# soulslicer/probabilistic-depth

Hardware: AMD Instinct MI355X
Metric: depth-volumes/sec (D=64, 256x512) (higher is better)
Workload: dtype f32 (fp16-pair products on MFMA, fp32 accumulate)

## Files before the change

probabilistic-depth_amd/csrc/sweep_dist.hip:

```cpp
#include <hip/hip_runtime.h>

#include <atomic>
#include <climits>
#include <cstdlib>

#include "dist_layout.hpp"
#include "epipolar_probe.hpp"
#include "geometry.hpp"
#include "kernels.hpp"
#include "sweep_workspace.hpp"
#include "wave_util.hpp"

#include "sweep_dist_knobs.hpp"

namespace pdepth {

namespace {

using namespace wv;
typedef _Float16 h8 __attribute__((ext_vector_type(8)));
typedef _Float16 h2 __attribute__((ext_vector_type(2)));
typedef int v2i __attribute__((ext_vector_type(2)));

constexpr int DIST_MAXV = 8;

struct DistArgs {
    SweepArgs a;
    const char* packed;
    const float* stats;
    int* queue;
    int* qcnt;
    int qstride;
    int tiles_x, ntile;
    int one_each;
    int nblk;
    int nonce;
};
#define KARG(type, field) kernarg_at<type>(offsetof(DistArgs, field))


__device__ __forceinline__ float dist_exp(float x) {
    return __builtin_amdgcn_exp2f((x < -1000.0f ? -1000.0f : x) * 1.44269502162933349609375f);
}

template <int MAXB, int NAC>
struct __attribute__((aligned(16))) DistLds {
    static constexpr int XSTRIDE = MAXB * 16 + 4;
    float Ys[16 * XSTRIDE];
    float Qs[(MAXB + 3) / 4 * 256 + 8];
    _Float16 Bs[NAC * 4 * 16 * 8];
    float rp[4 * 16 * 2];
    float mus[dist::MAX_C + 8];
    float xf[DIST_MAXV * 12];
    float cst[8];
    float red[4 * 16 * 4];
    float dcl[128];
    int ctab[2][64 * 2];
    int ired[2][2];
    int brow[MAXB + 2];
    v4i rec[2];
    int iflag;
    unsigned char wide[64];
};

template <int NCHK, int NH>
__global__ __launch_bounds__(256, NH == 1 ? DIST_OCC1 : DIST_OCC2) void sweep_dist_kernel(DistArgs da) {
    constexpr int NAC = 2 * NCHK + 1;
    constexpr int MP = NCHK + 1;
    constexpr int MAXB = NH == 1 ? DIST_MAXB1 : DIST_MAXB2;
    constexpr int NC = 4 * NH;
    constexpr int QPL = 8 * NCHK + 3;
    constexpr int NS = NH == 1 ? DIST_SETS1 : DIST_SETS2;
    typedef DistLds<MAXB, NAC> Lds;
    constexpr int XSTRIDE = Lds::XSTRIDE;
    __shared__ Lds L;
#ifdef DIST_STAMPS
    unsigned long long stamp_acc[12] = {0, 0, 0, 0, 0, 0, 0, 0, 0, 0, 0, 0};
    unsigned long long stamp_t = __builtin_amdgcn_s_memtime();
#endif
    if (poison_on_foreign_layout(da.a, da.queue, LAYOUT_DIST16)) return;
    const int tid = threadIdx.x;
    constexpr int QT = 64 * DIST_QUEUE_WAVE;
    static_assert(DIST_QUEUE_WAVE >= 0 && DIST_QUEUE_WAVE < 4, "a workgroup has four waves");

    {
        const float* dc = KARG(const float*, a.d_candi);
        const int D = KARG(int, a.D);
        for (int k = tid; k < 64 * NH; k += 256) L.dcl[k] = dc[min(k, D - 1)];
    }
    if (tid < 128) { L.ctab[0][tid] = (tid & 1) ? INT_MIN : INT_MAX; L.ctab[1][tid] = (tid & 1) ? INT_MIN : INT_MAX; }
    if (tid < 64) L.wide[tid] = 1;
    if (tid < 2) { L.ired[tid][0] = INT_MAX; L.ired[tid][1] = INT_MIN; }
    __syncthreads();
    if ((int)(tid >> 2) < min(KARG(int, a.B), 64) && epipolar_probe_is_steep(da.a, tid >> 2, tid & 3)) L.wide[tid >> 2] = 0;

    const int xcd = blockIdx.x & 7;
    if (blockIdx.x == 0 && tid == 0) KARG(int*, queue)[DIST_NONCE_SLOT] = KARG(int, nonce);
    auto band_tiles_of = [&](int q) { const int nt = KARG(int, ntile); return (nt >> 3) + (q < (nt & 7) ? 1 : 0); };
    auto band_first_of = [&](int q) {
        const int nt = KARG(int, ntile), qq = nt >> 3, rr8 = nt & 7;
        return q < rr8 ? q * (qq + 1) : rr8 * (qq + 1) + (q - rr8) * qq;
    };
    auto items_of = [&](int q) { return 4 * band_tiles_of(q) * KARG(int, a.B); };
    int own_done = 0;
    auto steal = [&]() -> int {
        int* qcnt = KARG(int*, qcnt);
        const int qs = KARG(int, qstride);
#pragma unroll 1
        for (int j = 1; j < 8; ++j) {
            const int q = (opaque_s(xcd) + j) & 7, nq = items_of(q);
            if (__hip_atomic_load(&qcnt[q * qs], __ATOMIC_RELAXED, __HIP_MEMORY_SCOPE_AGENT) >= nq) continue;
            const int got = atomicAdd(&qcnt[q * qs], 1);
            if (got < nq) return (q << 28) | got;
        }
        return -1;
    };
    auto resolve = [&](int got) -> int {
        const int n_own = items_of(xcd);
        if (!own_done && got < n_own) return (opaque_s(xcd) << 28) | got;
        own_done = 1;
        return steal();
    };
    auto fdiv = [](int nn, int dd) { return (int)(((float)nn + 0.5f) * __builtin_amdgcn_rcpf((float)dd)); };
    auto decode = [&](int item, int& b_, int& tx_, int& ty_, int& sub_) {
        const int ntile = KARG(int, ntile), tiles_x = KARG(int, tiles_x), H = KARG(int, a.H);
        const int qq = ntile >> 3, rr8 = ntile & 7;
        const bool small_idx = (long long)ntile * 4 * KARG(int, a.B) < (1ll << 22);
        const int tiles_y_ = (H + 3) / 4;
        const int q_ = item >> 28, iq = item & 0x0fffffff, band_tiles = band_tiles_of(q_);
        const int tidx = iq >> 2;
        sub_ = iq & 3;
        b_ = small_idx ? fdiv(tidx, band_tiles) : tidx / band_tiles;
        const int ti = tidx - b_ * band_tiles;
        int tile = band_first_of(q_) + ti;
        if (rr8 == 0 && tiles_y_ % 16 == 0 && tiles_y_ * tiles_x == ntile) {
            const int hb_rows = tiles_y_ / 16, half_tiles = hb_rows * tiles_x;
            const int second = ti >= half_tiles ? 1 : 0, tih = ti - second * half_tiles;
            const int hbi = (q_ < 4) == (second == 0) ? q_ : 8 + q_;
            const int cc = small_idx ? fdiv(tih, hb_rows) : tih / hb_rows, r_ = tih - cc * hb_rows;
            tile = (hbi * hb_rows + r_) * tiles_x + cc;
        } else if (rr8 == 0 && qq % tiles_x == 0) {
            const int band_rows = qq / tiles_x, tc = small_idx ? fdiv(ti, band_rows) : ti / band_rows;
            tile = (q_ * band_rows + (ti - tc * band_rows)) * tiles_x + tc;
        }
        ty_ = small_idx ? fdiv(tile, tiles_x) : tile / tiles_x;
        tx_ = tile - ty_ * tiles_x;
        if (DIST_REV_BATCH && KARG(const float*, a.src) != nullptr) b_ = KARG(int, a.B) - 1 - b_;
    };
#define ONE_EACH (KARG(int, one_each) != 0)
    __syncthreads();

    int state = 0;
    int n_direct = 0;
    int got_own = (tid == QT && !ONE_EACH) ? atomicAdd(&KARG(int*, qcnt)[xcd * KARG(int, qstride)], 1) : (int)(blockIdx.x >> 3);
    int next_item = -1;
    auto resolve_next = [&]() { if (opaque_v((int)threadIdx.x) == QT) next_item = ONE_EACH ? -1 : resolve(got_own); };
    constexpr int REC_WIDE = 1, REC_BELOW = 2, REC_FIRST = 4;
    auto publish = [&](int slot, int item) {
        v4i r = v4i{item, 0, 0, 0};
        if (item >= 0) {
            int b, tx, ty, sub;
            decode(item, b, tx, ty, sub);
            const bool wide = b < 64 ? L.wide[b] != 0 : false;
            const int x0 = wide ? tx * 16 : tx * 16 + 8 * (sub & 1), y0 = wide ? ty * 4 + sub : ty * 4 + 2 * (sub >> 1);
            r.y = b;
            r.z = (y0 << 16) | x0;
            r.w = (wide ? REC_WIDE : 0) | (y0 >= KARG(int, a.H) ? REC_BELOW : 0) | ((tx | ty | sub) == 0 ? REC_FIRST : 0);
        }
        L.rec[slot] = r;
    };
    constexpr bool EARLY = DIST_DECODE_EARLY != 0;
    constexpr bool POP_EARLY = EARLY && DIST_PREFETCH == 0;
    auto record_next = [&](bool decode = true, bool pop = true) {
        if (opaque_v((int)threadIdx.x) == QT) {
            if (decode) publish(state & 1, next_item);
            if (pop && POP_EARLY && !ONE_EACH && !own_done) got_own = atomicAdd(&KARG(int*, qcnt)[xcd * KARG(int, qstride)], 1);
        }
    };
    auto publish_next = [&]() {
        if (opaque_v((int)threadIdx.x) == QT) {
            if (!EARLY) publish(state & 1, next_item);
            if (!POP_EARLY && !ONE_EACH && !own_done) got_own = atomicAdd(&KARG(int*, qcnt)[xcd * KARG(int, qstride)], 1);
        }
    };
    constexpr bool PF = DIST_PREFETCH != 0;
    constexpr int ZW = 64 + 128 * NCHK;
    static_assert(4 * ZW + 128 <= (int)(sizeof(Lds::Qs) / sizeof(float)), "the prefetch zone does not fit L.Qs");
    auto dma_pixels = [&](int wave, int b, int p4) {
        const int H = KARG(int, a.H), W = KARG(int, a.W), C = KARG(int, a.C), HW = H * W;
        const int kq = (opaque_v((int)threadIdx.x) & 63) >> 4;
        const __amdgpu_buffer_rsrc_t rray =
            __builtin_amdgcn_make_buffer_rsrc((void*)(KARG(const float*, a.rays) + (size_t)b * 3 * HW), 0, 3 * HW * 4, 0x00020000);
        const __amdgpu_buffer_rsrc_t rref = __builtin_amdgcn_make_buffer_rsrc(
            (void*)(KARG(const float*, a.ref) + (size_t)b * KARG(long long, a.ref_bstride)), 0, C * HW * 4, 0x00020000);
        dma_b32(rray, lds_addr_of(&L.Qs[wave * ZW]), kq < 3 ? kq * HW * 4 + p4 : OOB, 0);
#pragma unroll
        for (int mm = 0; mm < NCHK; ++mm)
#pragma unroll
            for (int j = 0; j < 2; ++j) {
                const int cr = 8 * wave + 4 * j + kq;
                dma_b32(rref, lds_addr_of(&L.Qs[wave * ZW + 64 + 128 * mm + 64 * j]), cr < C - 32 * mm ? cr * HW * 4 + p4 : OOB, 32 * mm * HW * 4);
            }
        if (wave == 0) {
#pragma unroll
            for (int j = 0; j < 2; ++j) {
                const int cr = 4 * j + kq;
                dma_b32(rref, lds_addr_of(&L.Qs[4 * ZW + 64 * j]), cr < C - 32 * NCHK ? cr * HW * 4 + p4 : OOB, 32 * NCHK * HW * 4);
            }
        }
    };
    auto prefetch_next = [&](int wave) {
        const v4i nrec = L.rec[state & 1];
        if (__builtin_amdgcn_readfirstlane(nrec.x) < 0) return;
        const int fl = __builtin_amdgcn_readfirstlane(nrec.w);
        if (fl & REC_BELOW) return;
        const int b = __builtin_amdgcn_readfirstlane(nrec.y), xy = __builtin_amdgcn_readfirstlane(nrec.z);
        const int H = KARG(int, a.H), W = KARG(int, a.W);
        const int n = opaque_v((int)threadIdx.x) & 15;
        const int x = (xy & 0xffff) + ((fl & REC_WIDE) ? n : (n & 7));
        const int y = (xy >> 16) + ((fl & REC_WIDE) ? 0 : (n >> 3));
        dma_pixels(wave, b, (min(y, H - 1) * W + min(x, W - 1)) * 4);
        state |= 4;
    };
    if (tid == QT) {
        publish(0, ONE_EACH ? (got_own < items_of(xcd) ? (xcd << 28) | got_own : -1) : resolve(got_own));
        if (!ONE_EACH && !own_done) got_own = atomicAdd(&KARG(int*, qcnt)[xcd * KARG(int, qstride)], 1);
    }
    PDEPTH_LDS_BARRIER();
#define PDEPTH_POP_WAIT(n) __builtin_amdgcn_s_waitcnt(0x0f70 | (n))
    PDEPTH_POP_WAIT(0);

    for (;;) {
        const v4i rec = L.rec[state & 1];
        state ^= 1;
        const int pf = state & 4;
        state ^= pf;
        if (__builtin_amdgcn_readfirstlane(rec.x) < 0) break;
        DSTAMP(0)
        const int wave = opaque_s(__builtin_amdgcn_readfirstlane((int)threadIdx.x >> 6));
        const int b = __builtin_amdgcn_readfirstlane(rec.y), xy0 = __builtin_amdgcn_readfirstlane(rec.z), recfl = __builtin_amdgcn_readfirstlane(rec.w);
        const int H = KARG(int, a.H), W = KARG(int, a.W), V = KARG(int, a.V), C = KARG(int, a.C), D = KARG(int, a.D);
        const bool wide = (recfl & REC_WIDE) != 0;

        {
            if (recfl & REC_BELOW) {
                resolve_next();
                if (EARLY) record_next();
                publish_next();
                PDEPTH_LDS_BARRIER();
                PDEPTH_POP_WAIT(0);
                continue;
            }
            const int tid = opaque_v((int)threadIdx.x), lane = tid & 63;
            const int n = lane & 15, kq = lane >> 4, tq = wave * 4 + kq;
            const int a32 = (lane ^ 32) << 2;
            const int HW = H * W;
            int p;
            bool xlive;
            float ray[3], rv[MP][2];
            {
                const __amdgpu_buffer_rsrc_t rray =
                    __builtin_amdgcn_make_buffer_rsrc((void*)(KARG(const float*, a.rays) + (size_t)b * 3 * HW), 0, 3 * HW * 4, 0x00020000);
                const __amdgpu_buffer_rsrc_t rref = __builtin_amdgcn_make_buffer_rsrc(
                    (void*)(KARG(const float*, a.ref) + (size_t)b * KARG(long long, a.ref_bstride)), 0, C * HW * 4, 0x00020000);
                const int x = (xy0 & 0xffff) + (wide ? n : (n & 7));
                const int y = (xy0 >> 16) + (wide ? 0 : (n >> 3));
                xlive = x < W && y < H;
                p = min(y, H - 1) * W + min(x, W - 1);
                if (PF) {
                    if (!pf) dma_pixels(wave, b, p * 4);
                } else {
#pragma unroll
                    for (int i = 0; i < 3; ++i) ray[i] = __builtin_bit_cast(float, __builtin_amdgcn_raw_buffer_load_b32(rray, p * 4, i * HW * 4, 0));
#pragma unroll
                    for (int mm = 0; mm < MP; ++mm) {
                        const bool mine = mm < NCHK || wave == 0;
#pragma unroll
                        for (int i = 0; i < 2; ++i)
                            rv[mm][i] = __builtin_bit_cast(float, __builtin_amdgcn_raw_buffer_load_b32(
                                rref, mine && 2 * tq + i < C - 32 * mm ? ((2 * tq + i) * HW + p) * 4 : OOB, 32 * mm * HW * 4, 0));
                    }
                }
            }
            if (DIST_DECODE_EARLY == 1) { resolve_next(); record_next(); }
            DSTAMP(1)
            const bool new_b = b + 1 != state >> 3;
            if (new_b) {
                state = (state & 7) | ((b + 1) << 3);
                const int tid = opaque_v((int)threadIdx.x), lane = tid & 63;
                const float* st = KARG(const float*, stats) + (size_t)b * STATS_STRIDE;
                if (wave == 0) {
                    float am = st[STATS_AMAX + lane], sv = st[STATS_VAR + lane], sl_ = st[STATS_LAG + lane], m2 = st[lane] * st[lane];
                    if (lane + 64 < STATS_VAR) {
                        am = fmaxf(am, st[STATS_AMAX + lane + 64]); sv += st[STATS_VAR + lane + 64]; sl_ += st[STATS_LAG + lane + 64];
                        m2 += st[lane + 64] * st[lane + 64];
                    }
                    float dhi = fabsf(L.dcl[lane]), dlo = -dhi;
                    if (NH == 2) { const float d2 = fabsf(L.dcl[lane + 64]); dhi = fmaxf(dhi, d2); dlo = fmaxf(dlo, -d2); }
                    {
                        const int x32 = (lane ^ 32) << 2;
                        am = fmaxf(am, bperm_f(x32, am)); sv += bperm_f(x32, sv); sl_ += bperm_f(x32, sl_); m2 += bperm_f(x32, m2);
                        dhi = fmaxf(dhi, bperm_f(x32, dhi)); dlo = fmaxf(dlo, bperm_f(x32, dlo));
#define PDEPTH_XOR_STEP(M) { const int pat = ((M) << 10) | 0x1f; \
                             am = fmaxf(am, __builtin_bit_cast(float, __builtin_amdgcn_ds_swizzle(__builtin_bit_cast(int, am), pat))); \
                             sv += __builtin_bit_cast(float, __builtin_amdgcn_ds_swizzle(__builtin_bit_cast(int, sv), pat)); \
                             sl_ += __builtin_bit_cast(float, __builtin_amdgcn_ds_swizzle(__builtin_bit_cast(int, sl_), pat)); \
                             m2 += __builtin_bit_cast(float, __builtin_amdgcn_ds_swizzle(__builtin_bit_cast(int, m2), pat)); \
                             dhi = fmaxf(dhi, __builtin_bit_cast(float, __builtin_amdgcn_ds_swizzle(__builtin_bit_cast(int, dhi), pat))); \
                             dlo = fmaxf(dlo, __builtin_bit_cast(float, __builtin_amdgcn_ds_swizzle(__builtin_bit_cast(int, dlo), pat))); }
                        PDEPTH_XOR_STEP(16) PDEPTH_XOR_STEP(8) PDEPTH_XOR_STEP(4) PDEPTH_XOR_STEP(2) PDEPTH_XOR_STEP(1)
#undef PDEPTH_XOR_STEP
                    }
                    const int e = dist::scale_exponent(am);
                    const float sc = ldexpf(1.0f, e);
                    const float sg = KARG(float, a.sigma);
                    const bool outside = sv > DIST_GUARD_RATIO * sl_ && sv * 10.0f > DIST_GUARD_ENERGY * fabsf(sg);
                    const bool illcond = (float)KARG(int, a.V) * (2.0f * sv + m2) * (dhi + dlo) * 1.1920929e-7f > PDEPTH_COND_LIMIT * fabsf(sg);
                    if (lane == 0) {
                        L.cst[6] = sc; L.cst[7] = ldexpf(refined_rcp(sg), -2 * e);
                        const int pf = reinterpret_cast<const int*>(st + STATS_FLAGS)[0];
                        L.iflag = (pf != 0 ? 1 : 0) | (outside ? 2 : 0) | (illcond ? 4 : 0);
                    }
                    for (int c = lane; c < dist::MAX_C + 8; c += 64) L.mus[c] = st[c] * sc;
                }
                if (tid >= 128 && tid < 128 + V) {
                    const int v = tid - 128;
                    ViewXform xf;
                    make_view_xform(KARG(const float*, a.K) + b * 9, KARG(const float*, a.R) + ((size_t)b * V + v) * 9,
                                    KARG(const float*, a.t) + ((size_t)b * V + v) * 3, KARG(int, a.blas_mode), xf);
    #pragma unroll
                    for (int i = 0; i < 9; ++i) L.xf[v * 12 + i] = xf.kr[i];
    #pragma unroll
                    for (int i = 0; i < 3; ++i) L.xf[v * 12 + 9 + i] = xf.kt[i];
                }
                if (tid == 255) {
                    const float* const cxcy_ = KARG(const float*, a.cxcy);
                    const float cx = cxcy_[b * 2 + 0], cy = cxcy_[b * 2 + 1];
                    L.cst[0] = cx; L.cst[1] = cy; L.cst[2] = refined_rcp(cx); L.cst[3] = refined_rcp(cy);
                    L.cst[4] = (float)W / 2.0f; L.cst[5] = (float)H / 2.0f;
                }
            }
            bool item_ready = !new_b;
            if (KARG(const float*, a.src) != nullptr) {
                if (!item_ready) { PDEPTH_LDS_BARRIER(); item_ready = true; }
                if ((__builtin_amdgcn_readfirstlane(L.iflag) & 7) != 0) {
                    if (opaque_v((int)threadIdx.x) == QT && (recfl & REC_FIRST)) {
                        reinterpret_cast<int*>(const_cast<float*>(KARG(const float*, stats)) + (size_t)b * STATS_STRIDE + STATS_FLAGS)[1] = 1;
                        n_direct += KARG(int, tiles_x) * (wide ? H : 2 * ((H + 1) >> 1));
                    }
                    if (DIST_DECODE_EARLY != 1) resolve_next();
                    if (DIST_DECODE_EARLY == 2) record_next();
                    publish_next();
                    PDEPTH_LDS_BARRIER();
                    PDEPTH_POP_WAIT(0);
                    continue;
                }
            }
            float rr = 0.0f, zc = 0.0f;
            bool centred = false;
            unsigned failmask = 0;
            float cost[NC];
#pragma unroll
            for (int j = 0; j < NC; ++j) cost[j] = 0.0f;
            if (PF) {
                if (pf && (KARG(float*, a.logp_out) != nullptr || KARG(float*, a.depth_out) != nullptr)) {
                    if (NC == 4) asm volatile("s_waitcnt vmcnt(4)" ::: "memory");
                    else asm volatile("s_waitcnt vmcnt(8)" ::: "memory");
                } else {
                    asm volatile("s_waitcnt vmcnt(0)" ::: "memory");
                }
                const float* const z = &L.Qs[wave * ZW];
#pragma unroll
                for (int i = 0; i < 3; ++i) ray[i] = z[16 * i + n];
#pragma unroll
                for (int mm = 0; mm < MP; ++mm)
#pragma unroll
                    for (int i = 0; i < 2; ++i)
                        rv[mm][i] = mm < NCHK ? z[64 + 128 * mm + 16 * (2 * kq + i) + n] : (wave == 0 ? L.Qs[4 * ZW + 16 * (2 * kq + i) + n] : 0.0f);
            }

            constexpr bool RETRY = NH == 2;
            for (int v = 0; v < V; ++v) {
                const char* const srcv_v = RETRY ? nullptr : KARG(const char*, packed) + (size_t)((size_t)b * V + v) * dist::view_bytes(C, H, W);
                const int H_ = H, W_ = W, C_ = C, D_ = D;
#pragma unroll
                for (int h = 0; h < NH; ++h) {
                    if (!item_ready) { PDEPTH_LDS_BARRIER(); item_ready = true; }
                    int attempt = 0;
                    for (;;) {
                    const bool mine = attempt == 0 || (wave >> 1) == attempt - 1;
                    const int H = RETRY ? KARG(int, a.H) : H_, W = RETRY ? KARG(int, a.W) : W_, C = RETRY ? KARG(int, a.C) : C_, D = RETRY ? KARG(int, a.D) : D_;
                    int cell[4];
                    float fw[4], fn[4];
                    {
                        ViewXform xf;
                        {
                            const v4f k0 = *reinterpret_cast<const v4f*>(&L.xf[v * 12]), k1 = *reinterpret_cast<const v4f*>(&L.xf[v * 12 + 4]),
                                      k2 = *reinterpret_cast<const v4f*>(&L.xf[v * 12 + 8]);
                            xf.kr[0] = k0.x; xf.kr[1] = k0.y; xf.kr[2] = k0.z; xf.kr[3] = k0.w; xf.kr[4] = k1.x; xf.kr[5] = k1.y;
                            xf.kr[6] = k1.z; xf.kr[7] = k1.w; xf.kr[8] = k2.x; xf.kt[0] = k2.y; xf.kt[1] = k2.z; xf.kt[2] = k2.w;
                            xf.separate = KARG(int, a.blas_mode);
                        }
                        const v4f c0 = *reinterpret_cast<const v4f*>(&L.cst[0]);
                        const v2f c1 = *reinterpret_cast<const v2f*>(&L.cst[4]);
                        const v4f dk = *reinterpret_cast<const v4f*>(&L.dcl[64 * h + 4 * tq]);
                        float t2a, t2b, t2c;
                        ray_term2(xf, ray[0], ray[1], ray[2], t2a, t2b, t2c);
#pragma unroll
                        for (int j = 0; j < 4; ++j) {
                            const int k = 64 * h + 4 * tq + j;
                            float ix, iy;
                            plane_sample_pos_fast(xf, t2a, t2b, t2c, dk[j], c0.x, c0.y, c0.z, c0.w, c1.x, c1.y, ix, iy);
                            cell[j] = cell_of(ix, iy, W, H, fw[j], fn[j]);
                            if (k >= D || !xlive || !mine) cell[j] = NO_CELL;
                        }
#pragma unroll
                        for (int j = 0; j < 4; ++j) { asm volatile("" : "+v"(fw[j])); asm volatile("" : "+v"(fn[j])); }
                    }
                    DSTAMP(2)
                    if (!centred) {
                        const float sc = L.cst[6], sm2 = -2.0f * sc;
                        float pr = 0.0f, pz = 0.0f;
                        int* const Bw = reinterpret_cast<int*>(L.Bs);
#pragma unroll
                        for (int mm = 0; mm < MP; ++mm) {
                            if (mm == NCHK && wave != 0) continue;
                            const v2f mu2 = *reinterpret_cast<const v2f*>(&L.mus[32 * mm + 2 * tq]);
                            const float x0 = __builtin_fmaf(rv[mm][0], sm2, 2.0f * mu2.x), x1 = __builtin_fmaf(rv[mm][1], sm2, 2.0f * mu2.y);
                            const float s0 = rv[mm][0] * sc, s1 = rv[mm][1] * sc;
                            pr = __builtin_fmaf(x0, x0, pr); pr = __builtin_fmaf(x1, x1, pr);
                            pz = __builtin_fmaf(s0, s0, pz); pz = __builtin_fmaf(s1, s1, pz);
                            const h2 bh = __builtin_convertvector(v2f{x0, x1}, h2);
                            const h2 bl = __builtin_convertvector(v2f{x0 - (float)bh.x, x1 - (float)bh.y}, h2);
                            if (mm < NCHK) {
                                Bw[((mm * 4 + wave) * 16 + n) * 4 + kq] = __builtin_bit_cast(int, bh);
                                Bw[(((NCHK + mm) * 4 + wave) * 16 + n) * 4 + kq] = __builtin_bit_cast(int, bl);
                            } else {
                                Bw[(((2 * NCHK) * 4 + 0) * 16 + n) * 4 + kq] = __builtin_bit_cast(int, bh);
                                Bw[(((2 * NCHK) * 4 + 1) * 16 + n) * 4 + kq] = __builtin_bit_cast(int, bh);
                                Bw[(((2 * NCHK) * 4 + 2) * 16 + n) * 4 + kq] = __builtin_bit_cast(int, bl);
                            }
                        }
                        pr = 0.25f * pr;
                        pr = pr + xor16_f(pr); pr = pr + bperm_f(a32, pr);
                        pz = pz + xor16_f(pz); pz = pz + bperm_f(a32, pz);
                        if (kq == 0) *reinterpret_cast<v2f*>(&L.rp[(wave * 16 + n) * 2]) = v2f{pr, pz};
                    }
                    const int par = (state >> 1) & 1;
                    {
                        int ylo = 32767, yhi = -32768;
                        int rmin = 0, rmax = 0, ry = 0;
                        bool open = false;
#pragma unroll
                        for (int j = 0; j < 4; ++j) {
                            const bool vj = cell[j] != NO_CELL;
                            const int yj = cell_y(cell[j]), xj = cell_x(cell[j]);
                            const bool cont = open && vj && yj == ry;
                            if (open && !cont) {
                                atomicMin(&L.ctab[par][(ry & 63) * 2], rmin);
                                atomicMax(&L.ctab[par][(ry & 63) * 2 + 1], rmax);
                            }
                            rmin = cont ? min(rmin, xj) : xj;
                            rmax = cont ? max(rmax, xj) : xj;
                            ry = yj;
                            open = vj;
                            ylo = min(ylo, vj ? yj : 32767);
                            yhi = max(yhi, yj);
                        }
                        if (open) {
                            atomicMin(&L.ctab[par][(ry & 63) * 2], rmin);
                            atomicMax(&L.ctab[par][(ry & 63) * 2 + 1], rmax);
                        }
                        const int wmin = wave_min_i(ylo), wmax = wave_max_i(yhi);
                        if (lane == 0 && wmin <= wmax) { atomicMin(&L.ired[par][0], wmin); atomicMax(&L.ired[par][1], wmax); }
                    }
                    DSTAMP(3)
                    PDEPTH_LDS_BARRIER();
                    DSTAMP(4)
                    if (!centred) {
#pragma unroll
                        for (int w = 0; w < 4; ++w) {
                            const v2f pp = *reinterpret_cast<const v2f*>(&L.rp[(w * 16 + n) * 2]);
                            rr = rr + pp.x; zc = zc + pp.y;
                        }
                        if (kq == 3) {
                            const dist::Pieces pq = dist::split_pieces(rr < 2.0e9f ? rr : __builtin_nanf(""));
                            h8 sp;
                            sp[0] = (_Float16)dist::PIECE_C1; sp[1] = (_Float16)dist::PIECE_C2; sp[2] = (_Float16)dist::PIECE_C3;
                            sp[3] = pq.p1; sp[4] = pq.p2; sp[5] = pq.p3; sp[6] = (_Float16)0.f; sp[7] = (_Float16)0.f;
                            *reinterpret_cast<h8*>(&L.Bs[(((NAC - 1) * 4 + 3) * 16 + n) * 8]) = sp;
                        }
                        centred = true;
                    }
                    h8 Bv[NAC];
                    const _Float16* const bsl = &L.Bs[(kq * 16 + n) * 8];
#pragma unroll
                    for (int i = 0; i < NAC; ++i) Bv[i] = *reinterpret_cast<const h8*>(bsl + i * 512);
                    const int yb = __builtin_amdgcn_readfirstlane(L.ired[par][0]), yt = __builtin_amdgcn_readfirstlane(L.ired[par][1]);
                    int nb = 0, lo = 0, nblk = 0, fb = 0;
                    bool fits = true;
                    if (yb <= yt) {
                        const int ncell = yt - yb + 1;
                        if (ncell + 1 > 64 || ncell + 1 > MAXB) {
                            fits = false;
                        } else {
                            const v2i e0 = *reinterpret_cast<const v2i*>(&L.ctab[par][((yb + lane) & 63) * 2]);
                            const v2i e1 = *reinterpret_cast<const v2i*>(&L.ctab[par][((yb + lane - 1) & 63) * 2]);
                            const int l0 = min(e0.x, e1.x), h0 = max(e0.y, e1.y);
                            lo = ((l0 + dist::RING) & ~3) - dist::RING;
                            nblk = l0 <= h0 ? (h0 - lo + 2 + 15) >> 4 : 0;
                            const int incl = wave_scan_incl(nblk);
                            nb = __builtin_amdgcn_readlane(incl, 63);
                            fits = nb <= MAXB;
                            fb = incl - nblk;
                        }
                    }
                    const int iflag = __builtin_amdgcn_readfirstlane(L.iflag);
                    if ((iflag & 3) != 0) fits = false;
                    if (DIST_FORCE_DIRECT == -1 || DIST_FORCE_DIRECT == v) fits = false;
                    state ^= 2;
                    const int rowoff = 16 * fb - lo;
                    const bool go = fits && nb > 0;
                    DSTAMP(5)
                    int sl0[4], sl1[4];
                    {
                        constexpr int PB = dist::GROUP_PLANE_BYTES, GB = (8 * NCHK + 4) * PB;
                        const int Wp = dist::wp(W);
                        const int ntex = (n / dist::GROUP) * GB + (n % dist::GROUP) * 16;
                        const char* srcv = RETRY ? KARG(const char*, packed) + (size_t)((size_t)b * KARG(int, a.V) + v) * dist::view_bytes(C, H, W) : srcv_v;
                        const __amdgpu_buffer_rsrc_t rsrc = __builtin_amdgcn_make_buffer_rsrc((void*)srcv, 0, (int)dist::view_bytes(C, H, W), 0x00020000);
                        const int voffA = opaque_v(ntex + kq * PB);
                        h8 S[NS][NAC];
                        int boff = 0;
                        if (go) {
#pragma unroll 1
                            for (int i = 0; i < nblk; ++i) L.brow[fb + i] = lane;
                            const int rho = L.brow[min(lane, MAXB - 1)];
                            const int xs = __builtin_amdgcn_ds_bpermute(4 * rho, lo) + 16 * (lane - __builtin_amdgcn_ds_bpermute(4 * rho, fb));
                            boff = lane < nb ? ((yb + rho + dist::RING) * (Wp / dist::GROUP) + (xs + dist::RING) / dist::GROUP) * GB : OOB;
                        }
                        auto fetch = [&S, rsrc, voffA](int set, int i, int soff) {
                            int voff = voffA;
                            if (i == NAC - 1) {
                                static_assert(PB == 64 && GB % 256 == 0, "kq = bits 6..7 of voffA");
                                asm volatile("" : "+v"(voff));
                                voff -= (int)((0x40800000u >> ((voff >> 3) & 0x18)) & 0xffu);
                            }
                            S[set][i] = __builtin_bit_cast(h8, __builtin_amdgcn_raw_buffer_load_b128(rsrc, voff, soff + i * 4 * PB, 0));
                        };
                        auto fetch_block = [&](int set, int soff) {
#pragma unroll
                            for (int c = 0; c < NCHK; ++c) { fetch(set, c, soff); fetch(set, NCHK + c, soff); }
                            fetch(set, NAC - 1, soff);
                        };
                        const bool decode_here = DIST_DECODE_EARLY == 2 && v == 0 && h == 0 && attempt == 0;
                        const int wsh = DIST_DECODE_EARLY == 2 ? (wave + 3 - DIST_QUEUE_WAVE) & 3 : wave;
                        const int q = (nb + 3) >> 2, b0 = wsh * q, b1 = min(nb, b0 + q);
                        __builtin_amdgcn_s_setprio(1);
                        if (go) {
#pragma unroll
                            for (int u = 0; u < NS; ++u)
                                if (b0 + u < b1) fetch_block(u, __builtin_amdgcn_readlane(boff, b0 + u));
#pragma unroll
                            for (int gq = 0; gq < (MAXB + 15) / 16; ++gq) {
                                const int g = wave + 4 * gq;
                                if (4 * g < nb) {
                                    const int bo = __builtin_amdgcn_ds_bpermute(4 * (4 * g + kq), boff);
                                    const int vq = 4 * g + kq < nb ? bo + ntex : OOB;
                                    dma_b128(rsrc, lds_addr_of(&L.Qs[g * 256]), vq, QPL * PB);
                                }
                            }
                        }
#pragma unroll
                        for (int j = 0; j < 4; ++j) {
                            const bool has = fits && cell[j] != NO_CELL;
                            const int r = has ? cell_y(cell[j]) - yb : 0;
                            const int o0 = __builtin_amdgcn_ds_bpermute(4 * r, rowoff), o1 = __builtin_amdgcn_ds_bpermute(4 * r + 4, rowoff);
                            const int cxx = cell_x(cell[j]);
                            sl0[j] = has ? cxx + o0 : -1;
                            sl1[j] = cxx + o1;
                        }
                        if (go) {
                            auto y_block = [&](int u, int bj, bool more) {
                                const int soff = more ? __builtin_amdgcn_readlane(boff, bj + NS) : 0;
                                v4f acc = v4f{0.f, 0.f, 0.f, 0.f};
#pragma unroll
                                for (int c = 0; c < NCHK; ++c) {
                                    acc = __builtin_amdgcn_mfma_f32_16x16x32_f16(S[u][c], Bv[c], acc, 0, 0, 0);
                                    acc = __builtin_amdgcn_mfma_f32_16x16x32_f16(S[u][c], Bv[NCHK + c], acc, 0, 0, 0);
                                    if (more) fetch(u, c, soff);
                                    acc = __builtin_amdgcn_mfma_f32_16x16x32_f16(S[u][NCHK + c], Bv[c], acc, 0, 0, 0);
                                    if (more) fetch(u, NCHK + c, soff);
                                }
                                acc = __builtin_amdgcn_mfma_f32_16x16x32_f16(S[u][NAC - 1], Bv[NAC - 1], acc, 0, 0, 0);
                                if (more) fetch(u, NAC - 1, soff);
                                int bjo = bj;
                                asm volatile("" : "+s"(bjo));
                                *reinterpret_cast<v4f*>(&L.Ys[n * XSTRIDE + 16 * bjo + 4 * kq]) = acc;
                            };
                            int bi = b0;
#pragma unroll 1
                            for (; bi + 2 * NS <= b1; bi += NS) {
#pragma unroll
                                for (int u = 0; u < NS; ++u) y_block(u, bi + u, true);
                            }
                            if (bi < b1) {
                                if (NS == 1) {
                                    y_block(0, bi, false);
                                } else {
                                    y_block(0, bi, bi + 2 < b1);
                                    if (bi + 1 < b1) y_block(1, bi + 1, false);
                                    if (bi + 2 < b1) y_block(0, bi + 2, false);
                                }
                            }
                            DSTAMP(6)
                        }
                        if (decode_here) { resolve_next(); record_next(true, false); }
                        if (go) asm volatile("s_waitcnt vmcnt(0)" ::: "memory");
                        if (decode_here) record_next(false, true);
                        __builtin_amdgcn_s_setprio(0);
                    }
                    DSTAMP(7)
                    PDEPTH_LDS_BARRIER();
                    DSTAMP(8)
                    if (wave == 1) {
                        *reinterpret_cast<v2i*>(&L.ctab[par][lane * 2]) = v2i{INT_MAX, INT_MIN};
                        if (lane == 0) { L.ired[par][0] = INT_MAX; L.ired[par][1] = INT_MIN; }
                    }

                    if (!fits) {
                        if (attempt != 0) failmask |= 1u << ((v * NH + h) * 2 + attempt - 1);
                    } else if (attempt == 0 || (wave >> 1) == attempt - 1) {
                        const float cinv = L.cst[7];
                        const float* yr = &L.Ys[n * XSTRIDE];
#pragma unroll
                        for (int j = 0; j < 4; ++j) {
                            float qv = zc + (fw[j] + fn[j]) * 0.0f;
                            if (sl0[j] >= 0) {
                                const int s0 = sl0[j], s1 = sl1[j];
                                const float Y00 = yr[s0], Y01 = yr[s0 + 1], Y10 = yr[s1], Y11 = yr[s1 + 1];
                                const v4f qa = *reinterpret_cast<const v4f*>(&L.Qs[s0 * 4]);
                                const float dy1 = L.Qs[s0 * 4 + 5];
                                const float ex = 1.0f - fw[j], ey = 1.0f - fn[j];
                                const float w00 = ey * ex, w01 = ey * fw[j], w10 = fn[j] * ex, w11 = fn[j] * fw[j];
                                const float ys = __builtin_fmaf(w11, Y11, __builtin_fmaf(w10, Y10, __builtin_fmaf(w01, Y01, w00 * Y00)));
                                const float qi = __builtin_fmaf(w11, qa.z, __builtin_fmaf(w10, qa.y, w01 * qa.x));
                                const float qo = __builtin_fmaf(w01, dy1, w10 * qa.w);
                                qv = ys - __builtin_fmaf(w11, qo, w00 * qi);
                            }
                            cost[4 * h + j] = cost[4 * h + j] + qv * cinv;
                        }
                    }
                    DSTAMP(9)
                    if (!RETRY) {
                        if (!fits) failmask |= 3u << ((v * NH + h) * 2);
                        break;
                    }
                    if (attempt == 0) {
                        if (fits) break;
                        if ((iflag & 3) != 0 || DIST_FORCE_DIRECT == -1 || DIST_FORCE_DIRECT == v) {
                            failmask |= 3u << ((v * NH + h) * 2);
                            break;
                        }
                    } else if (attempt == 2) {
                        break;
                    }
                    ++attempt;
                    }
                }
            }

            if (failmask != 0) {
                const int H = KARG(int, a.H), W = KARG(int, a.W), V = KARG(int, a.V), C = KARG(int, a.C), D = KARG(int, a.D);
                const int b = opaque_s((state >> 3) - 1);
                const v4f c0 = *reinterpret_cast<const v4f*>(&L.cst[0]), c1 = *reinterpret_cast<const v4f*>(&L.cst[4]);
                const bool ovf = (L.iflag & 1) != 0;
                (void)0;
#pragma unroll 1
                for (int vhh = 0; vhh < V * NH * 2; ++vhh) {
                    if (!(failmask >> vhh & 1u)) continue;
                    if (tid == QT) ++n_direct;
                    if ((wave >> 1) != (vhh & 1)) continue;
                    const int vh = vhh >> 1, v = vh / NH, h = vh - v * NH;
                    ViewXform xf;
#pragma unroll
                    for (int i = 0; i < 9; ++i) xf.kr[i] = L.xf[v * 12 + i];
#pragma unroll
                    for (int i = 0; i < 3; ++i) xf.kt[i] = L.xf[v * 12 + 9 + i];
                    xf.separate = KARG(int, a.blas_mode);
                    float t2a, t2b, t2c;
                    ray_term2(xf, ray[0], ray[1], ray[2], t2a, t2b, t2c);
                    const char* srcv = KARG(const char*, packed) + (size_t)((size_t)b * V + v) * dist::view_bytes(C, H, W);
#pragma unroll 1
                    for (int j = 0; j < 4; ++j) {
                        const int k = 64 * h + 4 * tq + j;
                        float ix, iy, fwj, fnj;
                        plane_sample_pos_fast(xf, t2a, t2b, t2c, L.dcl[k], c0.x, c0.y, c0.z, c0.w, c1.x, c1.y, ix, iy);
                        int cellj = cell_of(ix, iy, W, H, fwj, fnj);
                        if (k >= D || !xlive) cellj = NO_CELL;
                        float qv = zc + (fwj + fnj) * 0.0f;
                        if (cellj != NO_CELL) {
                            const int cxx = cell_x(cellj), cyy = cell_y(cellj);
                            const float ex = 1.0f - fwj, ey = 1.0f - fnj;
                            const float w00 = ey * ex, w01 = ey * fwj, w10 = fnj * ex, w11 = fnj * fwj;
                            const long long t00 = dist::texel_offset(C, H, W, 0, cyy + dist::RING, cxx + dist::RING), t01 = dist::texel_offset(C, H, W, 0, cyy + dist::RING, cxx + dist::RING + 1);
                            const long long t10 = dist::texel_offset(C, H, W, 0, cyy + dist::RING + 1, cxx + dist::RING), t11 = dist::texel_offset(C, H, W, 0, cyy + dist::RING + 1, cxx + dist::RING + 1);
                            const long long pstep = dist::texel_offset(C, H, W, 1, 0, 0);
                            float part = 0.0f;
#pragma unroll 1
                            for (int g = 0; g < 4 * NCHK + 1; ++g) {
                                const bool tail = g == 4 * NCHK;
                                const char* ph = srcv + (tail ? 8 * NCHK : g) * pstep;
                                const char* pl = srcv + (tail ? 8 * NCHK + 1 : 4 * NCHK + g) * pstep;
                                const h8 a00 = *reinterpret_cast<const h8*>(ph + t00), a01 = *reinterpret_cast<const h8*>(ph + t01);
                                const h8 a10 = *reinterpret_cast<const h8*>(ph + t10), a11 = *reinterpret_cast<const h8*>(ph + t11);
                                const h8 l00 = *reinterpret_cast<const h8*>(pl + t00), l01 = *reinterpret_cast<const h8*>(pl + t01);
                                const h8 l10 = *reinterpret_cast<const h8*>(pl + t10), l11 = *reinterpret_cast<const h8*>(pl + t11);
                                const h8 rh = *reinterpret_cast<const h8*>(&L.Bs[(((tail ? 2 * NCHK : (g >> 2)) * 4 + (tail ? 0 : (g & 3))) * 16 + n) * 8]);
                                const h8 rl = *reinterpret_cast<const h8*>(&L.Bs[(((tail ? 2 * NCHK : NCHK + (g >> 2)) * 4 + (tail ? 2 : (g & 3))) * 16 + n) * 8]);
#pragma unroll
                                for (int i = 0; i < 8; ++i) {
                                    float val = ((float)a00[i] + (float)l00[i]) * w00;
                                    val = __builtin_fmaf((float)a01[i] + (float)l01[i], w01, val);
                                    val = __builtin_fmaf((float)a10[i] + (float)l10[i], w10, val);
                                    val = __builtin_fmaf((float)a11[i] + (float)l11[i], w11, val);
                                    const float rq = -0.5f * ((float)rh[i] + (float)rl[i]);
                                    const float diff = val - rq;
                                    part = __builtin_fmaf(diff, diff, part);
                                }
                            }
                            qv = part + (fwj + fnj) * 0.0f;
                        }
                        if (ovf) qv = __builtin_nanf("");
                        const float cj = qv * L.cst[7];
#pragma unroll
                        for (int jj = 0; jj < NC; ++jj) cost[jj] = cost[jj] + (jj == 4 * h + j ? cj : 0.0f);
                    }
                }
            }
            if (!EARLY) resolve_next();
            const int HW4 = KARG(int, a.H) * KARG(int, a.W) * 4;
            const int ovoff = xlive ? 4 * kq * HW4 + p * 4 : OOB;
            const int pl0 = 16 * wave * HW4;
            if (float* const cost_out = KARG(float*, a.cost_out)) {
                const __amdgpu_buffer_rsrc_t rc = __builtin_amdgcn_make_buffer_rsrc((void*)(cost_out + (size_t)b * D * (HW4 >> 2)), 0, D * HW4, 0x00020000);
#pragma unroll
                for (int j = 0; j < NC; ++j)
                    __builtin_amdgcn_raw_buffer_store_b32(__builtin_bit_cast(int, cost[j]), rc, ovoff, pl0 + (64 * (j >> 2) + (j & 3)) * HW4, 0);
            }
            float* const logp_out = KARG(float*, a.logp_out);
            float* const depth_out = KARG(float*, a.depth_out);
            if (logp_out || depth_out) {
                {
                    const int tq4 = opaque_v(4 * tq);
                    float mx = -INFINITY;
#pragma unroll
                    for (int j = 0; j < NC; ++j)
                        mx = max_raw(mx, 64 * (j >> 2) + tq4 + (j & 3) < D ? cost[j] : -INFINITY);
                    mx = max_raw(mx, xor16_f(mx));
                    mx = max_raw(mx, bperm_f(a32, mx));
                    float ssum = 0.0f, esum = 0.0f;
#pragma unroll
                    for (int j = 0; j < NC; ++j) {
                        const int k = 64 * (j >> 2) + tq4 + (j & 3);
                        const float ek = k < D ? dist_exp(cost[j] - mx) : 0.0f;
                        ssum = ssum + ek;
                        esum = __builtin_fmaf(L.dcl[k], ek, esum);
                    }
                    ssum = ssum + xor16_f(ssum); ssum = ssum + bperm_f(a32, ssum);
                    esum = esum + xor16_f(esum); esum = esum + bperm_f(a32, esum);
                    if (kq == 0) *reinterpret_cast<v4f*>(&L.red[(wave * 16 + n) * 4]) = v4f{mx, ssum, esum, 0.0f};
                }
                DSTAMP(10)
                publish_next();
                PDEPTH_LDS_BARRIER();
                {
                    v4f part[4];
#pragma unroll
                    for (int w = 0; w < 4; ++w) part[w] = *reinterpret_cast<const v4f*>(&L.red[(w * 16 + n) * 4]);
                    const float M = max_raw(max_raw(part[0].x, part[1].x), max_raw(part[2].x, part[3].x));
                    float S_ = 0.0f, E = 0.0f;
#pragma unroll
                    for (int w = 0; w < 4; ++w) {
                        const float scw = part[w].x == -INFINITY ? 0.0f : dist_exp(part[w].x - M);
                        S_ = __builtin_fmaf(part[w].y, scw, S_);
                        E = __builtin_fmaf(part[w].z, scw, E);
                    }
                    const float ls = logf(S_);
                    if (PF) { PDEPTH_POP_WAIT(0); prefetch_next(wave); }
                    {
                        const __amdgpu_buffer_rsrc_t rl = __builtin_amdgcn_make_buffer_rsrc(
                            (void*)(logp_out ? logp_out + (size_t)b * D * (HW4 >> 2) : nullptr), 0, logp_out ? D * HW4 : 0, 0x00020000);
#pragma unroll
                        for (int j = 0; j < NC; ++j)
                            __builtin_amdgcn_raw_buffer_store_b32(__builtin_bit_cast(int, (cost[j] - M) - ls), rl, ovoff,
                                                                  pl0 + (64 * (j >> 2) + (j & 3)) * HW4, 0);
                    }
                    if (depth_out && xlive && tq == 0) depth_out[(size_t)b * (HW4 >> 2) + p] = E / S_;
                }
                if (!PF) PDEPTH_POP_WAIT(NC);
            } else {
                publish_next();
                PDEPTH_LDS_BARRIER();
                PDEPTH_POP_WAIT(0);
                if (PF) prefetch_next(wave);
            }
            DSTAMP(11)
        }
    }
#undef PDEPTH_POP_WAIT
#ifdef DIST_STAMPS
    if ((threadIdx.x & 63) == 0 && (DIST_STAMP_WAVE < 0 || (int)(threadIdx.x >> 6) == DIST_STAMP_WAVE))
        for (int i = 0; i < 12; ++i) atomicAdd(reinterpret_cast<unsigned long long*>(KARG(int*, queue) + 8) + i, stamp_acc[i]);
#endif

    if (opaque_v((int)threadIdx.x) == QT) {
        int* queue = KARG(int*, queue);
        const int nonce = KARG(int, nonce);
        if (ONE_EACH) {
            if (n_direct) {
                int old = atomicAdd(&queue[DIST_DIRECT_LAST_SLOT], 0);
                for (;;) {
                    const int nv = (old >> 20) == nonce ? old + n_direct : (nonce << 20) | n_direct;
                    const int seen = atomicCAS(&queue[DIST_DIRECT_LAST_SLOT], old, nv);
                    if (seen == old) break;
                    old = seen;
                }
            }
        } else {
            if (n_direct) atomicAdd(&queue[DIST_DIRECT_SLOT], n_direct);
            const int done = atomicAdd(&queue[DIST_DONE_SLOT], 1);
            if (done == KARG(int, nblk) - 1) {
                const int nd = atomicAdd(&queue[DIST_DIRECT_SLOT], 0);
                for (int q = 0; q < 8; ++q) KARG(int*, qcnt)[q * KARG(int, qstride)] = 0;
                queue[DIST_DONE_SLOT] = 0;
                queue[DIST_DIRECT_SLOT] = 0;
                queue[DIST_DIRECT_LAST_SLOT] = (nonce << 20) | nd;
            }
        }
    }
}

inline int next_nonce() {
    static std::atomic<unsigned> launches{0};
    return (int)(launches.fetch_add(1) % 2047u) + 1;
}

template <int NCHK, int NH>
hipError_t launch_inst(const SweepArgs& a, const SweepWorkspace& ws, int tiles_x, int tiles, hipStream_t stream) {
    auto kern = sweep_dist_kernel<NCHK, NH>;
    static int per_cu[64] = {0};
    int dev = 0;
    if (hipGetDevice(&dev) != hipSuccess || dev < 0 || dev >= 64) dev = 0;
    if (per_cu[dev] == 0) {
        int nbk = 0;
        if (hipOccupancyMaxActiveBlocksPerMultiprocessor(&nbk, kern, 256, 0) != hipSuccess || nbk <= 0) nbk = 2;
        per_cu[dev] = nbk > 5 ? 5 : nbk;
    }
    long long nblk = ((long long)sweep_device_cus() * per_cu[dev] + 7) & ~7ll;
    DistArgs da;
    da.a = a; da.packed = ws.packed; da.stats = ws.stats; da.queue = ws.queue; da.tiles_x = tiles_x; da.ntile = tiles;
    int qs = DIST_QSTRIDE;
    while (qs * 8 > ws.nflags) qs >>= 1;
    da.qcnt = ws.dist_queue_counters();
    da.qstride = qs;
    da.nonce = next_nonce();
    const long long need = 8ll * ((tiles + 7) / 8) * 4 * a.B;
    da.one_each = need <= DIST_ONE_EACH_X * nblk;
    if (da.one_each) nblk = need;
    da.nblk = (int)nblk;
    hipLaunchKernelGGL(kern, dim3((unsigned)nblk), dim3(256), 0, stream, da);
    return hipGetLastError();
}

}

bool sweep_dist_supports(const SweepArgs& a) {
    const long long hw = (long long)a.H * a.W;
    return a.metric == 0 && a.D <= 128 && a.C <= dist::MAX_C && a.V <= DIST_MAXV && a.W <= 32760 && a.H <= 32760 &&
           hw * a.D * 4 < (1ll << 31) && hw * a.C * 4 < (1ll << 31) && dist::view_bytes(a.C, a.H, a.W) < (1ll << 31) && hw * 12 < (1ll << 31);
}

hipError_t launch_sweep_dist(const SweepArgs& a, void* workspace, hipStream_t stream, bool packed_ready) {
    const int tiles_x = (a.W + 15) / 16, tiles_y = (a.H + 3) / 4, tiles = tiles_x * tiles_y;
    const SweepWorkspace ws = SweepWorkspace::of(workspace, a);
    if (!packed_ready) {
        hipError_t e = launch_pack_dist(a, workspace, stream);
        if (e != hipSuccess) return e;
    }
    const int nck = dist::nchk(a.C);
    hipError_t e;
    if (a.D <= 64)
        e = nck == 0 ? launch_inst<0, 1>(a, ws, tiles_x, tiles, stream)
                     : (nck == 1 ? launch_inst<1, 1>(a, ws, tiles_x, tiles, stream) : launch_inst<2, 1>(a, ws, tiles_x, tiles, stream));
    else
        e = nck == 0 ? launch_inst<0, 2>(a, ws, tiles_x, tiles, stream)
                     : (nck == 1 ? launch_inst<1, 2>(a, ws, tiles_x, tiles, stream) : launch_inst<2, 2>(a, ws, tiles_x, tiles, stream));
    if (e != hipSuccess || a.src == nullptr) return e;
    return launch_sweep_direct_items(a, reinterpret_cast<const int*>(ws.stats + STATS_FLAGS) + 1, STATS_STRIDE, stream);
}

}
```

probabilistic-depth_amd/csrc/sweep_dist_knobs.hpp:

```cpp
#pragma once

#ifndef DIST_MAXB1
#define DIST_MAXB1 24
#endif
#ifndef DIST_MAXB2
#define DIST_MAXB2 34
#endif
#ifndef DIST_OCC1
#define DIST_OCC1 4
#endif
#ifndef DIST_OCC2
#define DIST_OCC2 3
#endif
#ifndef DIST_SETS1
#define DIST_SETS1 1
#endif
#ifndef DIST_SETS2
#define DIST_SETS2 2
#endif
#ifndef DIST_QSTRIDE
#define DIST_QSTRIDE 64
#endif
#ifndef DIST_PREFETCH
#define DIST_PREFETCH 0
#endif
#ifndef DIST_DECODE_EARLY
#define DIST_DECODE_EARLY 2
#endif
#ifndef DIST_QUEUE_WAVE
#define DIST_QUEUE_WAVE 3
#endif
#ifndef DIST_REV_BATCH
#define DIST_REV_BATCH 1
#endif
#ifndef DIST_ONE_EACH_X
#define DIST_ONE_EACH_X 6
#endif
#ifndef DIST_GUARD_RATIO
#define DIST_GUARD_RATIO 1.7f
#endif
#ifndef DIST_GUARD_ENERGY
#define DIST_GUARD_ENERGY 110.0f
#endif
#ifndef DIST_FORCE_DIRECT
#define DIST_FORCE_DIRECT -2
#endif

#ifndef DIST_STAMP_WAVE
#define DIST_STAMP_WAVE -1
#endif
#ifdef DIST_STAMPS
#define DSTAMP(i) { const unsigned long long t_ = __builtin_amdgcn_s_memtime(); stamp_acc[i] += t_ - stamp_t; stamp_t = t_; }
#elif defined(DIST_MARKS)
#define DSTAMP(i) asm volatile("; MARK " #i ::: "memory");
#else
#define DSTAMP(i)
#endif
```

Baseline: 11700.

## Issue first block fetches before pixel-operand setup and lane offset computation

Adds a DIST_FIRST_FETCH path, on by default, that computes each wave's first NS block offsets with scalar ballot and readlane, then issues their buffer loads before building the B operands and per-lane offsets. A sched_barrier pins this order so global load latency overlaps the LDS reads and the offset scan. It also removes the clamp on the exp argument, which drops one compare and select but could change results for very negative inputs.

```diff
diff --git a/probabilistic-depth_amd/csrc/sweep_dist.hip b/probabilistic-depth_amd/csrc/sweep_dist.hip
--- a/probabilistic-depth_amd/csrc/sweep_dist.hip
+++ b/probabilistic-depth_amd/csrc/sweep_dist.hip
@@ -40,7 +40,7 @@
 
 
 __device__ __forceinline__ float dist_exp(float x) {
-    return __builtin_amdgcn_exp2f((x < -1000.0f ? -1000.0f : x) * 1.44269502162933349609375f);
+    return __builtin_amdgcn_exp2f(x * 1.44269502162933349609375f);
 }
 
 template <int MAXB, int NAC>
@@ -477,27 +477,43 @@
                     DSTAMP(3)
                     PDEPTH_LDS_BARRIER();
                     DSTAMP(4)
-                    if (!centred) {
-#pragma unroll
-                        for (int w = 0; w < 4; ++w) {
-                            const v2f pp = *reinterpret_cast<const v2f*>(&L.rp[(w * 16 + n) * 2]);
-                            rr = rr + pp.x; zc = zc + pp.y;
-                        }
-                        if (kq == 3) {
-                            const dist::Pieces pq = dist::split_pieces(rr < 2.0e9f ? rr : __builtin_nanf(""));
-                            h8 sp;
-                            sp[0] = (_Float16)dist::PIECE_C1; sp[1] = (_Float16)dist::PIECE_C2; sp[2] = (_Float16)dist::PIECE_C3;
-                            sp[3] = pq.p1; sp[4] = pq.p2; sp[5] = pq.p3; sp[6] = (_Float16)0.f; sp[7] = (_Float16)0.f;
-                            *reinterpret_cast<h8*>(&L.Bs[(((NAC - 1) * 4 + 3) * 16 + n) * 8]) = sp;
-                        }
-                        centred = true;
-                    }
                     h8 Bv[NAC];
-                    const _Float16* const bsl = &L.Bs[(kq * 16 + n) * 8];
-#pragma unroll
-                    for (int i = 0; i < NAC; ++i) Bv[i] = *reinterpret_cast<const h8*>(bsl + i * 512);
-                    const int yb = __builtin_amdgcn_readfirstlane(L.ired[par][0]), yt = __builtin_amdgcn_readfirstlane(L.ired[par][1]);
-                    int nb = 0, lo = 0, nblk = 0, fb = 0;
+#define DIST_PIXEL_OPERANDS()                                                                                                   \
+                    if (!centred) {                                                                                             \
+                        _Pragma("unroll")                                                                                       \
+                        for (int w = 0; w < 4; ++w) {                                                                           \
+                            const v2f pp = *reinterpret_cast<const v2f*>(&L.rp[(w * 16 + n) * 2]);                              \
+                            rr = rr + pp.x; zc = zc + pp.y;                                                                     \
+                        }                                                                                                       \
+                        if (kq == 3) {                                                                                          \
+                            const dist::Pieces pq = dist::split_pieces(rr < 2.0e9f ? rr : __builtin_nanf(""));                  \
+                            h8 sp;                                                                                              \
+                            sp[0] = (_Float16)dist::PIECE_C1; sp[1] = (_Float16)dist::PIECE_C2; sp[2] = (_Float16)dist::PIECE_C3; \
+                            sp[3] = pq.p1; sp[4] = pq.p2; sp[5] = pq.p3; sp[6] = (_Float16)0.f; sp[7] = (_Float16)0.f;          \
+                            *reinterpret_cast<h8*>(&L.Bs[(((NAC - 1) * 4 + 3) * 16 + n) * 8]) = sp;                             \
+                        }                                                                                                       \
+                        centred = true;                                                                                         \
+                    }                                                                                                           \
+                    {                                                                                                           \
+                        const _Float16* const bsl = &L.Bs[(kq * 16 + n) * 8];                                                   \
+                        _Pragma("unroll")                                                                                       \
+                        for (int i = 0; i < NAC; ++i) Bv[i] = *reinterpret_cast<const h8*>(bsl + i * 512);                      \
+                    }
+                    if (!DIST_FIRST_FETCH) { DIST_PIXEL_OPERANDS() }
+                    int yb, yt, iflag = 0;
+                    const char* packed_p = nullptr;
+                    int nview_p = 0;
+                    if (DIST_FIRST_FETCH) {
+                        v2i yrange = *reinterpret_cast<const v2i*>(&L.ired[par][0]);
+                        int iflag_v = L.iflag;
+                        if (RETRY) { packed_p = KARG(const char*, packed); nview_p = KARG(int, a.V); }
+                        asm volatile("" : "+v"(yrange), "+v"(iflag_v));
+                        iflag = __builtin_amdgcn_readfirstlane(iflag_v);
+                        yb = __builtin_amdgcn_readfirstlane(yrange.x); yt = __builtin_amdgcn_readfirstlane(yrange.y);
+                    } else {
+                        yb = __builtin_amdgcn_readfirstlane(L.ired[par][0]); yt = __builtin_amdgcn_readfirstlane(L.ired[par][1]);
+                    }
+                    int nb = 0, lo = 0, nblk = 0, fb = 0, incl = 0;
                     bool fits = true;
                     if (yb <= yt) {
                         const int ncell = yt - yb + 1;
@@ -509,13 +525,13 @@
                             const int l0 = min(e0.x, e1.x), h0 = max(e0.y, e1.y);
                             lo = ((l0 + dist::RING) & ~3) - dist::RING;
                             nblk = l0 <= h0 ? (h0 - lo + 2 + 15) >> 4 : 0;
-                            const int incl = wave_scan_incl(nblk);
+                            incl = wave_scan_incl(nblk);
                             nb = __builtin_amdgcn_readlane(incl, 63);
                             fits = nb <= MAXB;
                             fb = incl - nblk;
                         }
                     }
-                    const int iflag = __builtin_amdgcn_readfirstlane(L.iflag);
+                    if (!DIST_FIRST_FETCH) iflag = __builtin_amdgcn_readfirstlane(L.iflag);
                     if ((iflag & 3) != 0) fits = false;
                     if (DIST_FORCE_DIRECT == -1 || DIST_FORCE_DIRECT == v) fits = false;
                     state ^= 2;
@@ -527,18 +543,21 @@
                         constexpr int PB = dist::GROUP_PLANE_BYTES, GB = (8 * NCHK + 4) * PB;
                         const int Wp = dist::wp(W);
                         const int ntex = (n / dist::GROUP) * GB + (n % dist::GROUP) * 16;
-                        const char* srcv = RETRY ? KARG(const char*, packed) + (size_t)((size_t)b * KARG(int, a.V) + v) * dist::view_bytes(C, H, W) : srcv_v;
+                        const char* srcv = RETRY ? (DIST_FIRST_FETCH ? packed_p : KARG(const char*, packed)) + (size_t)((size_t)b * (DIST_FIRST_FETCH ? nview_p : KARG(int, a.V)) + v) * dist::view_bytes(C, H, W) : srcv_v;
                         const __amdgpu_buffer_rsrc_t rsrc = __builtin_amdgcn_make_buffer_rsrc((void*)srcv, 0, (int)dist::view_bytes(C, H, W), 0x00020000);
                         const int voffA = opaque_v(ntex + kq * PB);
                         h8 S[NS][NAC];
+#define DIST_BLOCK_OFF(rho, xs) (((yb + (rho) + dist::RING) * (Wp / dist::GROUP) + ((xs) + dist::RING) / dist::GROUP) * GB)
                         int boff = 0;
-                        if (go) {
-#pragma unroll 1
-                            for (int i = 0; i < nblk; ++i) L.brow[fb + i] = lane;
-                            const int rho = L.brow[min(lane, MAXB - 1)];
-                            const int xs = __builtin_amdgcn_ds_bpermute(4 * rho, lo) + 16 * (lane - __builtin_amdgcn_ds_bpermute(4 * rho, fb));
-                            boff = lane < nb ? ((yb + rho + dist::RING) * (Wp / dist::GROUP) + (xs + dist::RING) / dist::GROUP) * GB : OOB;
-                        }
+#define DIST_LANE_OFFSETS()                                                                                                     \
+                        if (go) {                                                                                               \
+                            _Pragma("unroll 1")                                                                                 \
+                            for (int i = 0; i < nblk; ++i) L.brow[fb + i] = lane;                                               \
+                            const int rho = L.brow[min(lane, MAXB - 1)];                                                        \
+                            const int xs = __builtin_amdgcn_ds_bpermute(4 * rho, lo) + 16 * (lane - __builtin_amdgcn_ds_bpermute(4 * rho, fb)); \
+                            boff = lane < nb ? DIST_BLOCK_OFF(rho, xs) : OOB;                                                   \
+                        }
+                        if (!DIST_FIRST_FETCH) { DIST_LANE_OFFSETS() }
                         auto fetch = [&S, rsrc, voffA](int set, int i, int soff) {
                             int voff = voffA;
                             if (i == NAC - 1) {
@@ -557,10 +576,26 @@
                         const int wsh = DIST_DECODE_EARLY == 2 ? (wave + 3 - DIST_QUEUE_WAVE) & 3 : wave;
                         const int q = (nb + 3) >> 2, b0 = wsh * q, b1 = min(nb, b0 + q);
                         __builtin_amdgcn_s_setprio(1);
+                        if (DIST_FIRST_FETCH) {
+                            if (go) {
+#pragma unroll
+                                for (int u = 0; u < NS; ++u)
+                                    if (b0 + u < b1) {
+                                        const int rho = __builtin_ctzll(__builtin_amdgcn_ballot_w64(incl > b0 + u));
+                                        const int xs = __builtin_amdgcn_readlane(lo, rho) + 16 * (b0 + u - __builtin_amdgcn_readlane(fb, rho));
+                                        fetch_block(u, DIST_BLOCK_OFF(rho, xs));
+                                    }
+                            }
+                            __builtin_amdgcn_sched_barrier(0);
+                            DIST_PIXEL_OPERANDS()
+                            DIST_LANE_OFFSETS()
+                        }
                         if (go) {
-#pragma unroll
-                            for (int u = 0; u < NS; ++u)
-                                if (b0 + u < b1) fetch_block(u, __builtin_amdgcn_readlane(boff, b0 + u));
+                            if (!DIST_FIRST_FETCH) {
+#pragma unroll
+                                for (int u = 0; u < NS; ++u)
+                                    if (b0 + u < b1) fetch_block(u, __builtin_amdgcn_readlane(boff, b0 + u));
+                            }
 #pragma unroll
                             for (int gq = 0; gq < (MAXB + 15) / 16; ++gq) {
                                 const int g = wave + 4 * gq;
@@ -571,6 +606,9 @@
                                 }
                             }
                         }
+#undef DIST_PIXEL_OPERANDS
+#undef DIST_LANE_OFFSETS
+#undef DIST_BLOCK_OFF
 #pragma unroll
                         for (int j = 0; j < 4; ++j) {
                             const bool has = fits && cell[j] != NO_CELL;
diff --git a/probabilistic-depth_amd/csrc/sweep_dist_knobs.hpp b/probabilistic-depth_amd/csrc/sweep_dist_knobs.hpp
--- a/probabilistic-depth_amd/csrc/sweep_dist_knobs.hpp
+++ b/probabilistic-depth_amd/csrc/sweep_dist_knobs.hpp
@@ -33,6 +33,9 @@
 #ifndef DIST_REV_BATCH
 #define DIST_REV_BATCH 1
 #endif
+#ifndef DIST_FIRST_FETCH
+#define DIST_FIRST_FETCH 1
+#endif
 #ifndef DIST_ONE_EACH_X
 #define DIST_ONE_EACH_X 6
 #endif
```

Result: no change. 11800 (median of 6 runs) (+0.8%).
